# grantsrb/PyTorch-A2C

Measured on AMD Instinct MI355X. Metric: env-steps/sec (rollout+update), higher is better.
Workload: dtype f32

## Files before the change

### pytorch-a2c_amd/csrc/conv.hip

```cpp
#include <stdlib.h>
#include <algorithm>
#include <map>
#include <mutex>
#include "a2c_common.h"

bool c3_supported(const a2c_conv_desc* d, int kind);
size_t c3_prep_floats(const a2c_conv_desc* d, int kind);
int c3_prep(const a2c_conv_desc* d, int kind, const float* weight, float* out, hipStream_t st);
int c3_fwd(const a2c_conv_desc* d, const float* in, long in_bs, const float* frag, const float* bias, int relu, float* out,
           long out_bs, unsigned* signs, long signs_bs, int B, hipStream_t st);
int c3_bwd_data(const a2c_conv_desc* d, const float* dout, const float* frag, const float* mask, const unsigned* signs,
                long signs_bs, float* din, int B, hipStream_t st);
long c3_sign_words(const a2c_conv_desc* d);
bool c3_bwd_signs_supported(const a2c_conv_desc* d);
bool c3_bwd_mask_supported(const a2c_conv_desc* d);
bool c3w_supported(const a2c_conv_desc* d);
size_t c3w_ws_bytes(const a2c_conv_desc* d);
int c3w_bwd_weight(const a2c_conv_desc* d, const float* in, long in_bs, const float* dout, float* dW, float* db, int B, void* ws,
                   size_t ws_bytes, hipStream_t st);
bool c3_fwd_frames_supported(const a2c_conv_desc* d);
bool c3_chain_supported(const a2c_conv_desc* d, int n);
int c3_chain_fwd(const a2c_conv_desc* d, int n, const float* in, long in_bs, const float* const* frag, const float* const* bias,
                 int relu, float* const* out, const long* out_bs, unsigned* const* signs, const long* signs_bs, int B, hipStream_t st);
int c3_fwd_frames(const a2c_conv_desc* d, const unsigned char* f, long bs, long T, const int* nv, long nv_s, const float* frag,
// ... 2846 lines not shown
    } else {
    WS_STI(v0, 0) WS_STI(v1, 1) WS_STI(v2, 2) WS_STI(v3, 3) WS_STI(v4, 4) WS_STI(v5, 5) WS_STI(v6, 6)
    WS_STI(v7, 7) WS_STI(v8, 8) WS_STI(v9, 9) WS_STI(v10, 10) WS_STI(v11, 11) WS_STI(v12, 12) WS_STI(v13, 13)
    }
    __syncthreads();
    if (bco < p.Cout) {
      const float* __restrict__ pl = ldo + bco * p.PLANEo;
      float sb = 0.f;
      for (int i = bpart; i < NP; i += ST_NT / 16) sb += pl[i];
      dbacc += sb;
    }
#define WS_ROWS(R0, R1)                                                                                     \
    for (int rr = (R0); rr < (R1); ++rr) {                                                                  \
      const int r = 2 * rr + h;                                                                             \
      const float* __restrict__ arow = ldo + j * p.PLANEo + r * p.OW + kk;                                  \
      const float* __restrict__ brow = img + r * 4 * p.WP + boff;                                              \
      for (int c0 = 0; c0 < c4n; c0 += 5) {                                                                 \
        float av[5];                                                                                        \
        float4 bv[5];                                                                                       \
        _Pragma("unroll") for (int u = 0; u < 5; ++u) {                                                     \
          const int c4 = min(c0 + u, c4n - 1);                                                              \
          av[u] = (c0 + u < c4n) ? arow[4 * c4] : 0.f;                                                      \
          bv[u] = *reinterpret_cast<const float4*>(brow + 16 * c4);                                         \
        }                                                                                                   \
        _Pragma("unroll") for (int u = 0; u < 5; ++u) {                                                     \
          acc0 = __builtin_amdgcn_mfma_f32_16x16x4f32(av[u], bv[u].x, acc0, 0, 0, 0);                       \
          acc1 = __builtin_amdgcn_mfma_f32_16x16x4f32(av[u], bv[u].y, acc1, 0, 0, 0);                       \
          acc2 = __builtin_amdgcn_mfma_f32_16x16x4f32(av[u], bv[u].z, acc2, 0, 0, 0);                       \
          acc3 = __builtin_amdgcn_mfma_f32_16x16x4f32(av[u], bv[u].w, acc3, 0, 0, 0);                       \
        }                                                                                                   \
      }                                                                                                     \
    }
    if (U8) {
      const unsigned char* __restrict__ nus = fsrc(nn);
      nv = p.nvalid[nn];
      WS_LDD(d0, 0, ndsrc) WS_LDD(d1, 1, ndsrc) WS_LDD(d2, 2, ndsrc) WS_LDD(d3, 3, ndsrc) WS_LDU(g0, 0, nus) WS_LDU(g1, 1, nus)
      WS_ROWS(0, s1)
      WS_LDU(g2, 2, nus) WS_LDU(g3, 3, nus) WS_LDU(g4, 4, nus) WS_LDU(g5, 5, nus) WS_LDU(g6, 6, nus) WS_LDU(g7, 7, nus)
      WS_ROWS(s1, s2)
      WS_LDU(g8, 8, nus) WS_LDU(g9, 9, nus) WS_LDU(g10, 10, nus) WS_LDU(g11, 11, nus) WS_LDU(g12, 12, nus) WS_LDU(g13, 13, nus)
      WS_ROWS(s2, nrow)
    } else {
    WS_LDD(d0, 0, ndsrc) WS_LDD(d1, 1, ndsrc) WS_LDD(d2, 2, ndsrc) WS_LDD(d3, 3, ndsrc) WS_LDI(v0, 0, nsrc) WS_LDI(v1, 1, nsrc)
    WS_ROWS(0, s1)
    WS_LDI(v2, 2, nsrc) WS_LDI(v3, 3, nsrc) WS_LDI(v4, 4, nsrc) WS_LDI(v5, 5, nsrc) WS_LDI(v6, 6, nsrc) WS_LDI(v7, 7, nsrc)
    WS_ROWS(s1, s2)
    WS_LDI(v8, 8, nsrc) WS_LDI(v9, 9, nsrc) WS_LDI(v10, 10, nsrc) WS_LDI(v11, 11, nsrc) WS_LDI(v12, 12, nsrc) WS_LDI(v13, 13, nsrc)
    WS_ROWS(s2, nrow)
    }
  }
  __syncthreads();
  float* __restrict__ scr = lds;
  if (h == 1) {
    *reinterpret_cast<float4*>(scr + ((q * 4 + 0) * 64 + lane) * 4) = (float4){acc0[0], acc0[1], acc0[2], acc0[3]};
    *reinterpret_cast<float4*>(scr + ((q * 4 + 1) * 64 + lane) * 4) = (float4){acc1[0], acc1[1], acc1[2], acc1[3]};
    *reinterpret_cast<float4*>(scr + ((q * 4 + 2) * 64 + lane) * 4) = (float4){acc2[0], acc2[1], acc2[2], acc2[3]};
    *reinterpret_cast<float4*>(scr + ((q * 4 + 3) * 64 + lane) * 4) = (float4){acc3[0], acc3[1], acc3[2], acc3[3]};
  }
  float* __restrict__ red = lds + 4096;
  red[bpart * 16 + bco] = dbacc;
  __syncthreads();
  float* __restrict__ sl = p.slab + (long)blockIdx.x * ((long)p.Cout * p.K + p.Cout);
  if (h == 0) {
#pragma unroll
    for (int x = 0; x < 4; ++x) {
      const float4 o = *reinterpret_cast<const float4*>(scr + ((q * 4 + x) * 64 + lane) * 4);
      const f32x4 a = x == 0 ? acc0 : x == 1 ? acc1 : x == 2 ? acc2 : acc3;
      const float t[4] = {a[0] + o.x, a[1] + o.y, a[2] + o.z, a[3] + o.w};
#pragma unroll
      for (int rr = 0; rr < 4; ++rr) {
        const int co = 4 * kk + rr;
        if (co < p.Cout) sl[(long)co * p.K + knat + x] = t[rr];
      }
    }
  }
  if (tid < p.Cout) {
    float sb = 0.f;
    for (int x = 0; x < ST_NT / 16; ++x) sb += red[x * 16 + tid];
    sl[(long)p.Cout * p.K + tid] = sb;
  }
}

struct WsbGeo { int NG, NGT, NB, PA, PP, PLS, SK, no_ring; };
template <int DUMMY>
__global__ __launch_bounds__(ST_NT) __attribute__((amdgpu_waves_per_eu(2, 2))) void wgrad_stream_bf16_kernel(WstreamP p, WsbGeo gq) {
  extern __shared__ __attribute__((aligned(16))) float lds[];
  typedef __bf16 bf16x8w __attribute__((ext_vector_type(8)));
  unsigned short* __restrict__ A = reinterpret_cast<unsigned short*>(lds);
  unsigned short* __restrict__ P = A + 3 * 16 * gq.PA;
  const int tid = threadIdx.x, lane = tid & 63, w = tid >> 6;
  const int g = lane >> 4, j = lane & 15;
  const int HW = p.H * p.W, NP = p.OH * p.OW;
  const int w4 = p.W >> 2;
  const int dper4 = NP >> 2, dtot4 = p.Cout * dper4;
  const int NG = gq.NG, NGT = gq.NGT, NB = gq.NB, PA = gq.PA, PP = gq.PP, PLS = gq.PLS, SK = gq.SK;
  const int spr = (w4 + 1) >> 1, nslot = 4 * p.H * spr;
  {
    u32x4w* z = reinterpret_cast<u32x4w*>(lds);
    const int n16 = (3 * 16 * PA * 2 + 16 * PLS * 2) >> 4;
    for (int i = tid; i < n16; i += ST_NT) z[i] = (u32x4w){0u, 0u, 0u, 0u};
  }
  const int ky = j >> 1;
  f32x4 acc[16];
#pragma unroll
  for (int t = 0; t < 16; ++t) acc[t] = (f32x4){0.f, 0.f, 0.f, 0.f};
  float dbv[4] = {0.f, 0.f, 0.f, 0.f};
  f32x4 d0 = {}, d1 = {}, d2 = {}, d3 = {};
  uint2 g0 = {}, g1 = {}, g2 = {}, g3 = {}, g4 = {}, g5 = {}, g6 = {}, g7 = {};
  int nv = 4;
  auto fsrc = [&](long nn_) { const long r_ = nn_ / p.T; return p.fstore + r_ * p.fs_slot_stride + (nn_ - r_ * p.T) * (long)HW; };
  int soff[8];
  int sdst[8];
  unsigned int smask[8];
#pragma unroll
  for (int u = 0; u < 8; ++u) {
    const int idx = tid + u * ST_NT;
    const bool ok = idx < nslot;
    const int ii = ok ? idx : 0;
    const int c = ii / (p.H * spr), rem = ii - c * (p.H * spr), row = rem / spr, sp = rem - row * spr;
    soff[u] = (c * p.H + row) * p.W + 8 * sp;
    sdst[u] = ok ? (c * 4) * PLS + row * PP + (row >> 2) * SK + 2 * sp : -1;
    smask[u] = ((2 * sp + 1 < w4) ? 0xffffff00u : 0u) | (unsigned int)c;
  }
  int soff2[2], sdst2[2];
  unsigned int smask2[2];
#pragma unroll
  for (int u = 0; u < 2; ++u) {
    const int idx = tid + u * ST_NT;
    const bool ok = idx < p.H * spr;
    const int ii = ok ? idx : 0;
    const int row = ii / spr, sp = ii - row * spr;
    soff2[u] = (3 * p.H + row) * p.W + 8 * sp;
    sdst2[u] = ok ? row * PP + (row >> 2) * SK + 2 * sp : -1;
    smask2[u] = (2 * sp + 1 < w4) ? 1u : 0u;
  }
  int rot = 0;
  int pofs0 = 0, pofs1 = 4 * PLS, pofs2 = 8 * PLS, pofs3 = 12 * PLS;
  int adst[4];
#pragma unroll
  for (int u = 0; u < 4; ++u) {
    const int idx = tid + u * ST_NT;
    const bool ok = idx < dtot4;
    const int ii = ok ? idx : 0;
    const int co = ii / dper4, p0 = (ii - co * dper4) << 2;
    const int r = p0 / p.OW, c = p0 - r * p.OW;
    adst[u] = ok ? co * PA + (r * NG + (c >> 3)) * 8 + (c & 7) : -1;
  }
  const bool ring_off = gq.no_ring != 0;
  const long chunk = (p.B + gridDim.x - 1) / gridDim.x;
  long n = (long)blockIdx.x * chunk;
  const long n_end = n + chunk < (long)p.B ? n + chunk : (long)p.B;
#define WSB_LDU(var, u, src)                                                                                   \
  {                                                                                                            \
    const unsigned int* s_ = reinterpret_cast<const unsigned int*>((src) + soff[u]);                            \
    var.x = s_[0];                                                                                             \
    var.y = s_[(smask[u] >> 8) ? 1 : 0];                                                                       \
  }
#define WSB_LOADD(NN, D0, D1, D2, D3)                                                                          \
  {                                                                                                            \
    const float* __restrict__ ds_ = p.dout + (NN) * (long)p.Cout * NP;                                         \
    D0 = *reinterpret_cast<const f32x4*>(ds_ + (min(tid + 0 * ST_NT, dtot4 - 1) << 2));                        \
    D1 = *reinterpret_cast<const f32x4*>(ds_ + (min(tid + 1 * ST_NT, dtot4 - 1) << 2));                        \
    D2 = *reinterpret_cast<const f32x4*>(ds_ + (min(tid + 2 * ST_NT, dtot4 - 1) << 2));                        \
    D3 = *reinterpret_cast<const f32x4*>(ds_ + (min(tid + 3 * ST_NT, dtot4 - 1) << 2));                        \
  }
#define WSB_LDU2(var, u, src)                                                                                  \
  {                                                                                                            \
    const unsigned int* s_ = reinterpret_cast<const unsigned int*>((src) + soff2[u]);                           \
    var.x = s_[0];                                                                                             \
    var.y = s_[smask2[u] ? 1 : 0];                                                                             \
  }
#define WSB_LOADG(NN, INC_)                                                                                    \
  {                                                                                                            \
    const unsigned char* __restrict__ us_ = fsrc(NN);                                                          \
    if (INC_) {                                                                                                \
      WSB_LDU2(g0, 0, us_) WSB_LDU2(g1, 1, us_)                                                                \
    } else {                                                                                                   \
      WSB_LDU(g0, 0, us_) WSB_LDU(g1, 1, us_) WSB_LDU(g2, 2, us_) WSB_LDU(g3, 3, us_)                          \
      WSB_LDU(g4, 4, us_) WSB_LDU(g5, 5, us_) WSB_LDU(g6, 6, us_) WSB_LDU(g7, 7, us_)                          \
    }                                                                                                          \
  }
#define WSB_STD(var, u)                                                                                        \
  if (adst[u] >= 0) {                                                                                          \
    const float e_[4] = {var.x, var.y, var.z, var.w};                                                          \
    unsigned short pc_[3][4];                                                                                  \
    _Pragma("unroll") for (int i_ = 0; i_ < 4; ++i_) {                                                        \
      const __bf16 h0_ = (__bf16)e_[i_];                                                                       \
      const float r1_ = e_[i_] - (float)h0_;                                                                   \
      const __bf16 h1_ = (__bf16)r1_;                                                                          \
      const float r2_ = r1_ - (float)h1_;                                                                      \
      pc_[0][i_] = __builtin_bit_cast(unsigned short, h0_);                                                    \
      pc_[1][i_] = __builtin_bit_cast(unsigned short, h1_);                                                    \
      pc_[2][i_] = __builtin_bit_cast(unsigned short, (__bf16)r2_);                                            \
    }                                                                                                          \
    dbv[u] += (e_[0] + e_[1]) + (e_[2] + e_[3]);                                                               \
    unsigned short* a_ = A + adst[u];                                                                          \
    _Pragma("unroll") for (int pc = 0; pc < 3; ++pc)                                                          \
      *reinterpret_cast<uint2*>(a_ + pc * 16 * PA) = make_uint2((unsigned int)pc_[pc][0] | ((unsigned int)pc_[pc][1] << 16), \
                                                                (unsigned int)pc_[pc][2] | ((unsigned int)pc_[pc][3] << 16)); \
  }
#define WSB_STU(var, u)                                                                                        \
  if (sdst[u] >= 0) {                                                                                          \
    const int c_ = (int)(smask[u] & 0xffu);                                                                    \
    const unsigned int x0_ = c_ < 4 - nv ? 0u : var.x, x1_ = (c_ < 4 - nv || !(smask[u] >> 8)) ? 0u : var.y;   \
    unsigned int* d_ = reinterpret_cast<unsigned int*>(P + sdst[u]);                                           \
    const int ps_ = PLS >> 1;                                                                                  \
    d_[0] = __builtin_amdgcn_perm(__float_as_uint((float)(x1_ & 0xffu)), __float_as_uint((float)(x0_ & 0xffu)), 0x07060302u); \
    d_[ps_] = __builtin_amdgcn_perm(__float_as_uint((float)((x1_ >> 8) & 0xffu)), __float_as_uint((float)((x0_ >> 8) & 0xffu)), 0x07060302u); \
    d_[2 * ps_] = __builtin_amdgcn_perm(__float_as_uint((float)((x1_ >> 16) & 0xffu)), __float_as_uint((float)((x0_ >> 16) & 0xffu)), 0x07060302u); \
    d_[3 * ps_] = __builtin_amdgcn_perm(__float_as_uint((float)(x1_ >> 24)), __float_as_uint((float)(x0_ >> 24)), 0x07060302u); \
  }
  auto matrix = [&]() {
    for (int b = w; b < NB; b += ST_NT / 64) {
      const int grp = 4 * b + g;
      const unsigned short* __restrict__ ap = A + j * PA + grp * 8;
      const bf16x8w ah = *reinterpret_cast<const bf16x8w*>(ap);
      const bf16x8w am = *reinterpret_cast<const bf16x8w*>(ap + 16 * PA);
      const bf16x8w al = *reinterpret_cast<const bf16x8w*>(ap + 32 * PA);
      const int gcl = min(grp, NGT - 1);
      const int r = gcl / NG, gc = gcl - r * NG;
      const unsigned short* __restrict__ bp = P + (j & 1) * PLS + (4 * r + ky) * PP + (r + (ky >> 2)) * SK + 8 * gc;
#pragma unroll
      for (int t = 0; t < 16; ++t) {
        const int ci = t >> 2, kxh = (t >> 1) & 1, kp = t & 1;
        const int po = ci == 0 ? pofs0 : ci == 1 ? pofs1 : ci == 2 ? pofs2 : pofs3;
        const unsigned short* __restrict__ bx = bp + po + 2 * kp * PLS;
        const uint2 lo = *reinterpret_cast<const uint2*>(bx), hi = *reinterpret_cast<const uint2*>(bx + 4);
        u32x4w o;
        if (kxh) {
          const unsigned int nx = *reinterpret_cast<const unsigned int*>(bx + 8);
          o[0] = __builtin_amdgcn_alignbit(lo.y, lo.x, 16u);
          o[1] = __builtin_amdgcn_alignbit(hi.x, lo.y, 16u);
          o[2] = __builtin_amdgcn_alignbit(hi.y, hi.x, 16u);
          o[3] = __builtin_amdgcn_alignbit(nx, hi.y, 16u);
        } else {
          o[0] = lo.x; o[1] = lo.y; o[2] = hi.x; o[3] = hi.y;
        }
        const bf16x8w bv = __builtin_bit_cast(bf16x8w, o);
        acc[t] = __builtin_amdgcn_mfma_f32_16x16x32_bf16(ah, bv, acc[t], 0, 0, 0);
        acc[t] = __builtin_amdgcn_mfma_f32_16x16x32_bf16(am, bv, acc[t], 0, 0, 0);
        acc[t] = __builtin_amdgcn_mfma_f32_16x16x32_bf16(al, bv, acc[t], 0, 0, 0);
      }
    }
  };
#define WSB_STU2(var, u, PB_)                                                                                  \
  if (sdst2[u] >= 0) {                                                                                         \
    const unsigned int x0_ = var.x, x1_ = smask2[u] ? var.y : 0u;                                              \
    unsigned int* d_ = reinterpret_cast<unsigned int*>(P + (PB_) + sdst2[u]);                                  \
    const int ps_ = PLS >> 1;                                                                                  \
    d_[0] = __builtin_amdgcn_perm(__float_as_uint((float)(x1_ & 0xffu)), __float_as_uint((float)(x0_ & 0xffu)), 0x07060302u); \
    d_[ps_] = __builtin_amdgcn_perm(__float_as_uint((float)((x1_ >> 8) & 0xffu)), __float_as_uint((float)((x0_ >> 8) & 0xffu)), 0x07060302u); \
    d_[2 * ps_] = __builtin_amdgcn_perm(__float_as_uint((float)((x1_ >> 16) & 0xffu)), __float_as_uint((float)((x0_ >> 16) & 0xffu)), 0x07060302u); \
    d_[3 * ps_] = __builtin_amdgcn_perm(__float_as_uint((float)(x1_ >> 24)), __float_as_uint((float)(x0_ >> 24)), 0x07060302u); \
  }
  auto succ = [&](long a_, long b_, int nva_, int nvb_) {
    return !ring_off && b_ == a_ + 1 && (b_ % p.T) != 0 && nvb_ == 4 && nva_ >= 3;
  };
#define WSB_ITER(N_, D0, D1, D2, D3)                                                                           \
  {                                                                                                            \
    const long n2_ = ((N_) + 2 < n_end) ? (N_) + 2 : (N_);                                                     \
    const long n1_ = ((N_) + 1 < n_end) ? (N_) + 1 : (N_);                                                     \
    __syncthreads();                                  \
    if (inc_cur) rot = (rot + 1) & 3; else rot = 0;                                                            \
    pofs0 = rot * 4 * PLS; pofs1 = ((rot + 1) & 3) * 4 * PLS; pofs2 = ((rot + 2) & 3) * 4 * PLS; pofs3 = ((rot + 3) & 3) * 4 * PLS; \
    WSB_STD(D0, 0) WSB_STD(D1, 1) WSB_STD(D2, 2) WSB_STD(D3, 3)                                                \
    if (inc_cur) {                                                                                             \
      WSB_STU2(g0, 0, pofs3) WSB_STU2(g1, 1, pofs3)                                                            \
    } else {                                                                                                   \
      WSB_STU(g0, 0) WSB_STU(g1, 1) WSB_STU(g2, 2) WSB_STU(g3, 3) WSB_STU(g4, 4) WSB_STU(g5, 5) WSB_STU(g6, 6) WSB_STU(g7, 7) \
    }                                                                                                          \
    __syncthreads();                                                                                           \
                     \
    inc_cur = n1_ != (N_) && succ((N_), n1_, nv, nv1);                                                         \
    nv = nv1;                                             \
    WSB_LOADG(n1_, inc_cur)                                                                                    \
    nv1 = p.nvalid[n2_];                                                                                       \
    WSB_LOADD(n2_, D0, D1, D2, D3)                                                                             \
    matrix();                                                                                                  \
  }
  f32x4 e0 = {}, e1 = {}, e2 = {}, e3 = {};
  bool inc_cur = false;
  int nv1 = 4;
  if (n < n_end) {
    const long n1 = (n + 1 < n_end) ? n + 1 : n;
    WSB_LOADD(n, d0, d1, d2, d3)
    nv = p.nvalid[n];
    WSB_LOADG(n, false)
    nv1 = p.nvalid[n1];
    WSB_LOADD(n1, e0, e1, e2, e3)
  }
  for (; n < n_end; n += 2) {
    WSB_ITER(n, d0, d1, d2, d3)
    if (n + 1 < n_end) WSB_ITER(n + 1, e0, e1, e2, e3)
  }
#undef WSB_ITER
#undef WSB_STU2
#undef WSB_LDU2
#undef WSB_LOADD
#undef WSB_LOADG
#undef WSB_LDU
#undef WSB_STD
#undef WSB_STU
  float* __restrict__ sl = p.slab + (long)blockIdx.x * ((long)p.Cout * p.K + p.Cout);
  float* __restrict__ scr = lds;
#pragma unroll
  for (int t0 = 0; t0 < 16; t0 += 4) {
    __syncthreads();
#pragma unroll
    for (int x = 0; x < 4; ++x)
      *reinterpret_cast<float4*>(scr + ((w * 4 + x) * 64 + lane) * 4) = (float4){acc[t0 + x][0], acc[t0 + x][1], acc[t0 + x][2], acc[t0 + x][3]};
    __syncthreads();
#pragma unroll
    for (int e = 0; e < 2; ++e) {
      const int o = tid + e * ST_NT, x = o >> 8, l = (o >> 2) & 63, rr = o & 3;
      float v = scr[((0 * 4 + x) * 64 + l) * 4 + rr];
#pragma unroll
      for (int ww = 1; ww < ST_NT / 64; ++ww) v += scr[((ww * 4 + x) * 64 + l) * 4 + rr];
      const int t = t0 + x, ci = t >> 2, kxh = (t >> 1) & 1, kp = t & 1;
      const int jj = l & 15, co = 4 * (l >> 4) + rr;
      const int k = ((ci * 8 + (jj >> 1)) * 8) + 4 * kxh + 2 * kp + (jj & 1);
      if (co < p.Cout) sl[(long)co * p.K + k] = v;
    }
  }
  __syncthreads();
  float* __restrict__ red = lds;
#pragma unroll
  for (int u = 0; u < 4; ++u) red[tid + u * ST_NT] = dbv[u];
  __syncthreads();
  if (tid < p.Cout) {
    float sb = 0.f;
    for (int i = tid * dper4; i < (tid + 1) * dper4; ++i) sb += red[i];
    sl[(long)p.Cout * p.K + tid] = sb;
  }
}

static bool plan_wstream_bf16(const a2c_conv_desc* d, const WstreamP& p, WsbGeo& gq, size_t& lds) {
  gq.NG = (d->OW + 7) / 8;
  gq.no_ring = a2c_env_on("A2C_WSB_NO_RING");
  gq.NGT = d->OH * gq.NG;
  gq.NB = (gq.NGT + 3) / 4;
  const int need_dw = gq.NB * 16;
  int pa_dw = ((need_dw + 31) / 32) * 32 + 4;
  if (pa_dw - 32 >= need_dw) pa_dw -= 32;
  gq.PA = pa_dw * 2;
  gq.PP = gq.NG * 8 + 8;
  gq.SK = 4;
  gq.PLS = d->H * gq.PP + (d->H / 4 + 1) * gq.SK + 24;
  if (d->W / 4 > gq.NG * 8 + 1 || d->OW % 4 || d->Cout > 16) return false;
  lds = (size_t)3 * 16 * gq.PA * 2 + (size_t)16 * gq.PLS * 2;
  lds = (lds + 15) / 16 * 16;
  if (lds < 4 * (size_t)(8 * 4 * 256) || 4 * d->H * ((d->W / 4 + 1) / 2) > 8 * ST_NT) return false;
  if ((long)d->Cout * (d->OH * d->OW / 4) > 4L * ST_NT) return false;
  (void)p;
  return lds <= 160 * 1024 && (gq.PP * 2) % 8 == 0 && (gq.PLS * 2) % 8 == 0 && 4 * (d->OH - 1) + 7 < d->H;
}

static bool plan_wstream(const a2c_conv_desc* d, WstreamP& p) {
  if (!(d->ks == 8 && d->stride == 4 && d->pad == 0 && d->Cin == 4 && d->Cout <= 16 && d->W % 4 == 0 && d->OW % 4 == 0)) return false;
  const int NP = d->OH * d->OW;
  p.H = d->H; p.W = d->W; p.OH = d->OH; p.OW = d->OW; p.Cout = d->Cout; p.K = d->Cin * 64;
  p.WP = d->W;
  p.PLANE1 = ((d->H * p.WP + 63) / 64) * 64;
  p.PLANEo = ((NP + 31) / 32) * 32 + 2;
  if (d->H * d->W > ST_NS * ST_NT || d->Cout * NP > 4 * ST_NT * 4 || d->OH < 6) return false;
  if (4 * p.PLANE1 < 4096 + 512) return false;
  return 4 * (size_t)(4 * p.PLANE1 + 16 * p.PLANEo) <= 160 * 1024;
}
static int stream_grid() {
  static const int n_cu = []() { int dev = 0, n = 0; (void)hipGetDevice(&dev);
                                 (void)hipDeviceGetAttribute(&n, hipDeviceAttributeMultiprocessorCount, dev); return n > 0 ? n : 256; }();
  return n_cu;
}

__global__ __launch_bounds__(256) void wgrad_reduce_kernel(const float* __restrict__ slab, int nslab, long per,
                                                           long nW, float* __restrict__ dW, float* __restrict__ db) {
  for (long i = blockIdx.x * 256L + threadIdx.x; i < per; i += gridDim.x * 256L) {
    float s = 0.f;
    int z = 0;
    for (; z + 8 <= nslab; z += 8) {
      float t[8];
#pragma unroll
      for (int u = 0; u < 8; ++u) t[u] = slab[(long)(z + u) * per + i];
#pragma unroll
      for (int u = 0; u < 8; ++u) s += t[u];
    }
    for (; z < nslab; ++z) s += slab[(long)z * per + i];
    if (i < nW) dW[i] = s;
    else if (db) db[i - nW] = s;
  }
}

struct WgradPlan { SrcTile t; int OWp, PLANEo, MT, KTW, grid, run, rs, pf, ex; size_t lds; };

#define WGRAD_PF_A 1, 3, true, 4, 16, true
#define WGRAD_PF_C 2, 4, false, 12, 8, true
#define WGRAD_PF_D 2, 4, false, 14, 8, true, 2, 1
#define WGRAD_VARIANTS(X)                                                                                      \
  if (pl.pf == 2) { X(WGRAD_PF_D); }                                                                           \
  else if (pl.pf && pl.KTW == 3) { X(WGRAD_PF_A); }                                                            \
  else if (pl.pf) { X(WGRAD_PF_C); }                                                                           \
  else if (pl.rs && pl.KTW == 3) { X(1, 3, true, 0, 0, true); }                                                \
  else if (pl.rs) { X(2, 9, true, 0, 0, true); }                                                               \
  else if (pl.MT == 1 && pl.KTW == 1) { X(1, 1, false, 0, 0, true); }                                         \
  else if (pl.MT == 1 && pl.KTW == 4) { X(1, 4); }                                                            \
  else if (pl.MT == 2 && pl.KTW == 4 && pl.ex) { X(2, 4, false, 0, 0, true); }                                \
  else if (pl.MT == 2 && pl.KTW == 4) { X(2, 4); }                                                            \
  else if (pl.KTW == 5) { X(4, 5, false, 0, 0, true); }                                                       \
  else if (pl.ex) { X(4, 7, false, 0, 0, true); }                                                              \
  else { X(4, 7); }

static const void* wgrad_fn(const WgradPlan& pl) {
#define WGRAD_FN(...) return (const void*)wgrad_kernel<__VA_ARGS__>
  WGRAD_VARIANTS(WGRAD_FN)
#undef WGRAD_FN
}

static int wgrad_run_variant(const a2c_conv_desc* d) {
  if (!run_layout(d)) return 0;
  const int mt = ceil_div(d->Cout, 16), c4n = ceil_div(d->OW, 4), rgs = d->Cin * d->ks * 2 / 16;
  if (d->stride == 4 && mt == 1 && rgs == 4 && c4n == 5) return 1;
  if (d->stride == 2 && mt == 2 && rgs == 8 && c4n == 3) return 2;
  return 0;
}
// ... 818 lines not shown
    if (rc != A2C_OK) return rc;
  }
  return A2C_OK;
}
}
extern "C" {

size_t a2c_conv2d_bwd_data_w1_ws_bytes(const a2c_conv_desc* d2, const a2c_conv_desc* d1, int B) {
  BandW1Plan pl;
  if (B < 1 || !plan_band_w1(d2, d1, B, nullptr, pl)) return 0;
  int grid = 0;
  for (int v : {1, 2, 4}) {
    if (d2->OW % v) continue;
    pl.vec = v;
    const int g = band_w1_grid(pl, B);
    if (g > grid) grid = g;
  }
  return (size_t)grid * ((size_t)d1->Cout * d1->Cin * 9 + d1->Cout) * sizeof(float);
}

int a2c_conv2d_bwd_data_w1(const a2c_conv_desc* d2, const float* dout, const float* wprep_bwd, const float* mask,
                           const a2c_conv_desc* d1, const float* x, int64_t x_bstride, float* dW1, float* db1, int B,
                           void* ws, size_t ws_bytes, a2c_stream_t stream) {
  if (B < 1 || !dout || !wprep_bwd || !mask || !x || !dW1 || !db1) return A2C_ERR_ARG;
  BandW1Plan pl;
  if (((uintptr_t)mask % 16) || ((uintptr_t)x % 16) || x_bstride % 4 || !plan_band_w1(d2, d1, B, dout, pl)) return A2C_ERR_ARG;
  pl.q2.b.wfrag = wprep_bwd; pl.q2.b.mask = mask; pl.q2.b.din = nullptr;
  pl.fw.x = x; pl.fw.x_bs = x_bstride; pl.fw.slab = (float*)ws;
  const int grid = band_w1_grid(pl, B);
  const size_t per = (size_t)d1->Cout * pl.fw.K1 + d1->Cout;
  if (grid < 1) return A2C_ERR_ARG;
  if (!ws || ws_bytes < (size_t)grid * per * sizeof(float)) return A2C_ERR_WORKSPACE;
  hipStream_t st = a2c_s(stream);
#define W1_LAUNCH(V_, P_)                                                                                         \
  if (pl.vec == V_ && pl.pfb == P_)                                                                               \
    hipLaunchKernelGGL((bwd_band2_kernel<1, V_, P_, true>), dim3(grid), dim3(256), pl.lds, st, pl.q2, pl.fw);
  BAND_W1_CASES(W1_LAUNCH)
#undef W1_LAUNCH
  A2C_CHECK_LAUNCH();
  const long nW = (long)d1->Cout * pl.fw.K1;
  hipLaunchKernelGGL(wgrad_reduce_kernel, dim3(a2c_grid_1d((long)per, 256)), dim3(256), 0, st, (const float*)ws, grid,
                     (long)per, nW, dW1, db1);
  A2C_CHECK_LAUNCH();
  return A2C_OK;
}

size_t a2c_conv2d_bwd_weight_ws_bytes(const a2c_conv_desc* d, int B) {
  WgradPlan pl, pg;
  if (!desc_ok(d) || B < 0 || !plan_wgrad(d, B, pl) || !plan_wgrad(d, B, pg, false)) return 0;
  int grid = pl.grid > pg.grid ? pl.grid : pg.grid;
  WstreamP wp;
  if (plan_wstream(d, wp) && stream_grid() > grid) grid = stream_grid();
  const size_t base = (size_t)grid * ((size_t)d->Cout * d->Cin * d->ks * d->ks + d->Cout) * sizeof(float);
  const size_t c3 = c3w_ws_bytes(d);
  return c3 > base ? c3 : base;
}

int a2c_conv2d_bwd_weight_frames(const a2c_conv_desc* d, const uint8_t* fstore, int64_t slot_stride, int64_t T,
                                 const int* nvalid, const float* dout, float* dW, float* db, int B, void* ws, size_t ws_bytes,
                                 a2c_stream_t stream) {
  if (!desc_ok(d) || B < 1 || !fstore || !nvalid || !dout || !dW || T < 1) return A2C_ERR_ARG;
  if (c3w_supported(d) && d->Cin == 4) {
    if (((uintptr_t)fstore % 4) || slot_stride % 4 || ((uintptr_t)dout % 16) || ((uintptr_t)dW % 16) || ((uintptr_t)ws % 16) ||
        slot_stride < (T + 3) * (int64_t)d->H * d->W)
      return A2C_ERR_ARG;
    if (!ws || ws_bytes < a2c_conv2d_bwd_weight_ws_bytes(d, B)) return A2C_ERR_WORKSPACE;
    return c3w_bwd_weight_frames(d, fstore, (long)slot_stride, (long)T, nvalid, dout, dW, db, B, ws, ws_bytes, a2c_s(stream));
  }
  WstreamP wp;
  if (!plan_wstream(d, wp) || (d->H * d->W) % 16 || ((uintptr_t)fstore % 16) || slot_stride % 16 || ((uintptr_t)dout % 16) ||
      slot_stride < (T + 3) * (int64_t)d->H * d->W)
    return A2C_ERR_ARG;
  if (!ws || ws_bytes < a2c_conv2d_bwd_weight_ws_bytes(d, B)) return A2C_ERR_WORKSPACE;
  hipStream_t st = a2c_s(stream);
  const int grid = stream_grid();
  wp.in = nullptr; wp.in_bs = 0; wp.dout = dout; wp.slab = (float*)ws; wp.B = B;
  wp.fstore = fstore; wp.fs_slot_stride = (long)slot_stride; wp.T = (int)T; wp.nvalid = nvalid;
  {
    WsbGeo gq;
    size_t ldsb = 0;
    if (!a2c_env_on("A2C_WGRAD_F32") && plan_wstream_bf16(d, wp, gq, ldsb)) {
      static bool attrb = false;
      if (!attrb) {
        if (hipFuncSetAttribute((const void*)wgrad_stream_bf16_kernel<0>, hipFuncAttributeMaxDynamicSharedMemorySize, 160 * 1024) != hipSuccess)
          return A2C_ERR_LAUNCH;
        attrb = true;
      }
      const int gb = grid < B ? grid : B;
      hipLaunchKernelGGL(wgrad_stream_bf16_kernel<0>, dim3(gb), dim3(ST_NT), ldsb, st, wp, gq);
      A2C_CHECK_LAUNCH();
      const long nWb = (long)wp.Cout * wp.K, perb = nWb + wp.Cout;
      hipLaunchKernelGGL(wgrad_reduce_kernel, dim3(a2c_grid_1d(perb, 256)), dim3(256), 0, st, (const float*)ws, gb, perb, nWb, dW, db);
      A2C_CHECK_LAUNCH();
      return A2C_OK;
    }
  }
  const size_t lds = 4 * (size_t)(4 * wp.PLANE1 + 16 * wp.PLANEo);
  static bool attr = false;
  if (!attr) {
    if (hipFuncSetAttribute((const void*)wgrad_stream_kernel<true>, hipFuncAttributeMaxDynamicSharedMemorySize, 160 * 1024) != hipSuccess)
      return A2C_ERR_LAUNCH;
    attr = true;
  }
  hipLaunchKernelGGL(wgrad_stream_kernel<true>, dim3(grid < B ? grid : B), dim3(ST_NT), lds, st, wp);
  A2C_CHECK_LAUNCH();
  const int g = grid < B ? grid : B;
  const long nWs = (long)wp.Cout * wp.K, pers = nWs + wp.Cout;
  hipLaunchKernelGGL(wgrad_reduce_kernel, dim3(a2c_grid_1d(pers, 256)), dim3(256), 0, st, (const float*)ws, g, pers, nWs, dW, db);
  A2C_CHECK_LAUNCH();
  return A2C_OK;
}

int a2c_conv2d_bwd_weight_rank(const a2c_conv_desc* d, const float* in, int64_t in_bstride, const float* dl, int64_t ld_dl,
                               int n_logits, const float* Wc, const uint8_t* maskbits, int64_t mask_row_bytes, float* dW, float* db,
                               int B, void* ws, size_t ws_bytes, a2c_stream_t stream) {
  if (!desc_ok(d) || B < 1 || !in || !dl || !Wc || !maskbits || !dW || !db) return A2C_ERR_ARG;
  if (in_bstride % 4 || ((uintptr_t)in % 16) || ld_dl < n_logits || mask_row_bytes < (int64_t)d->Cout * d->OH * d->OW / 8 ||
      in_bstride < (int64_t)d->Cin * d->H * d->W || !a2c_conv2d_bwd_rank_supported(d, n_logits, B))
    return A2C_ERR_ARG;
  if (!ws || ws_bytes < a2c_conv2d_bwd_weight_ws_bytes(d, B)) return A2C_ERR_WORKSPACE;
  WgradPlan pl;
  if (!plan_wgrad(d, B, pl, true)) return A2C_ERR_ARG;
  const int grid = stream_grid() < pl.grid ? stream_grid() : pl.grid;
  hipStream_t st = a2c_s(stream);
  static bool attrr = false;
  if (!attrr) {
    if (hipFuncSetAttribute((const void*)wgrad_x6_kernel<true>, hipFuncAttributeMaxDynamicSharedMemorySize, wx::LDS_BYTES) != hipSuccess)
      return A2C_ERR_LAUNCH;
    attrr = true;
  }
  WgradX6P xp;
  xp.in = in; xp.in_bs = (long)in_bstride; xp.dout = nullptr; xp.slab = (float*)ws; xp.B = B;
  xp.dl = dl; xp.ldl = (long)ld_dl; xp.nlog = n_logits; xp.Wc = Wc; xp.a2b = maskbits; xp.a2b_row = (long)mask_row_bytes;
  hipLaunchKernelGGL(wgrad_x6_kernel<true>, dim3(grid), dim3(wx::NT), wx::LDS_BYTES, st, xp);
  A2C_CHECK_LAUNCH();
  const long nWx = 32L * 256, perx = nWx + 32;
  hipLaunchKernelGGL(wgrad_reduce_kernel, dim3(a2c_grid_1d(perx, 256)), dim3(256), 0, st, (const float*)ws, grid, perx, nWx, dW, db);
  A2C_CHECK_LAUNCH();
  return A2C_OK;
}

int a2c_conv2d_bwd_weight(const a2c_conv_desc* d, const float* in, int64_t in_bstride, const float* dout, float* dW,
                          float* db, int B, void* ws, size_t ws_bytes, a2c_stream_t stream) {
  WgradPlan pl;
  if (!desc_ok(d) || B < 1 || !in || !dout || !dW) return A2C_ERR_ARG;
  const bool aligned = (in_bstride % 4 == 0) && ((uintptr_t)in % 16 == 0) && ((uintptr_t)dout % 8 == 0);
  if (!plan_wgrad(d, B, pl, aligned)) return A2C_ERR_ARG;
  if (!ws || ws_bytes < a2c_conv2d_bwd_weight_ws_bytes(d, B)) return A2C_ERR_WORKSPACE;
  hipStream_t st = a2c_s(stream);
  if (c3w_supported(d) && aligned && ((uintptr_t)dout % 16 == 0) && ((uintptr_t)dW % 16 == 0) && ((uintptr_t)ws % 16 == 0))
    return c3w_bwd_weight(d, in, (long)in_bstride, dout, dW, db, B, ws, ws_bytes, st);
  {
    WstreamP wp;
    const int grid = stream_grid();
    if (aligned && B >= 8 * grid && ((uintptr_t)dout % 16 == 0) && !a2c_env_on("A2C_NO_STREAM") &&
        plan_wstream(d, wp)) {
      wp.in = in; wp.in_bs = in_bstride; wp.dout = dout; wp.slab = (float*)ws; wp.B = B;
      wp.fstore = nullptr; wp.fs_slot_stride = 0; wp.T = 1; wp.nvalid = nullptr;
      const size_t lds = 4 * (size_t)(4 * wp.PLANE1 + 16 * wp.PLANEo);
      static bool attr = false;
      if (!attr) {
        if (hipFuncSetAttribute((const void*)wgrad_stream_kernel<false>, hipFuncAttributeMaxDynamicSharedMemorySize, 160 * 1024) != hipSuccess)
          return A2C_ERR_LAUNCH;
        attr = true;
      }
      hipLaunchKernelGGL(wgrad_stream_kernel<false>, dim3(grid), dim3(ST_NT), lds, st, wp);
      A2C_CHECK_LAUNCH();
      const long nWs = (long)wp.Cout * wp.K, pers = nWs + wp.Cout;
      hipLaunchKernelGGL(wgrad_reduce_kernel, dim3(a2c_grid_1d(pers, 256)), dim3(256), 0, st, (const float*)ws, grid, pers, nWs,
                         dW, db);
      A2C_CHECK_LAUNCH();
      return A2C_OK;
// ... 59 lines not shown
```

Before: 10.07 million.

## Software-pipeline LDS reads in bf16 weight-grad MFMA loop with inline asm waits

Replaces the generic matrix() loop in the bf16 streaming weight-gradient kernel with a compile-time-unrolled pipeline. It prefetches A and B fragments from LDS with explicit ds_read instructions and uses fine-grained lgkmcnt waits so LDS latency overlaps the MFMA work. It also recomputes whole-frame staging addresses on the fly instead of keeping eight per-thread slot arrays and eight preloaded registers, which cuts register pressure. The old path stays selectable through an env var. The risks are fragile hand-scheduled waits, a new cap on block count that can reject some shapes, and extra code size from specialising each block count.

```diff
diff --git a/pytorch-a2c_amd/csrc/conv.hip b/pytorch-a2c_amd/csrc/conv.hip
--- a/pytorch-a2c_amd/csrc/conv.hip
+++ b/pytorch-a2c_amd/csrc/conv.hip
@@ -2952,7 +2952,31 @@
 }
 
 struct WsbGeo { int NG, NGT, NB, PA, PP, PLS, SK, no_ring; };
-template <int DUMMY>
+constexpr int WSB_MAXBLK = 4;
+typedef void __attribute__((address_space(3)))* wsb_lptr_t;
+__device__ __forceinline__ unsigned int wsb_lds_addr(const void* q) { return (unsigned int)(unsigned long)(wsb_lptr_t)q; }
+template <int OFF>
+__device__ __forceinline__ void wsb_read_a(u32x4w& v, unsigned int a) {
+  asm volatile("ds_read_b128 %0, %1 offset:%2" : "=v"(v) : "v"(a), "n"(OFF) : "memory");
+}
+__device__ __forceinline__ void wsb_read_b(u32x4w& v, unsigned int& t, unsigned int a) {
+  asm volatile("ds_read2_b64 %0, %1 offset1:1" : "=v"(v) : "v"(a) : "memory");
+  asm volatile("ds_read_b32 %0, %1 offset:16" : "=v"(t) : "v"(a) : "memory");
+}
+template <int N>
+__device__ __forceinline__ void wsb_wait(u32x4w& v, unsigned int& t) {
+  asm volatile("s_waitcnt lgkmcnt(%2)" : "+v"(v), "+v"(t) : "n"(N) : "memory");
+  __builtin_amdgcn_sched_barrier(0);
+}
+template <int N>
+__device__ __forceinline__ void wsb_wait(u32x4w& v, unsigned int& t, u32x4w& a0, u32x4w& a1, u32x4w& a2) {
+  asm volatile("s_waitcnt lgkmcnt(%5)" : "+v"(v), "+v"(t), "+v"(a0), "+v"(a1), "+v"(a2) : "n"(N) : "memory");
+  __builtin_amdgcn_sched_barrier(0);
+}
+template <int V>
+struct WsbC { static constexpr int value = V; };
+
+template <int SERIAL>
 __global__ __launch_bounds__(ST_NT) __attribute__((amdgpu_waves_per_eu(2, 2))) void wgrad_stream_bf16_kernel(WstreamP p, WsbGeo gq) {
   extern __shared__ __attribute__((aligned(16))) float lds[];
   typedef __bf16 bf16x8w __attribute__((ext_vector_type(8)));
@@ -2976,22 +3000,9 @@
   for (int t = 0; t < 16; ++t) acc[t] = (f32x4){0.f, 0.f, 0.f, 0.f};
   float dbv[4] = {0.f, 0.f, 0.f, 0.f};
   f32x4 d0 = {}, d1 = {}, d2 = {}, d3 = {};
-  uint2 g0 = {}, g1 = {}, g2 = {}, g3 = {}, g4 = {}, g5 = {}, g6 = {}, g7 = {};
+  uint2 g0 = {}, g1 = {};
   int nv = 4;
   auto fsrc = [&](long nn_) { const long r_ = nn_ / p.T; return p.fstore + r_ * p.fs_slot_stride + (nn_ - r_ * p.T) * (long)HW; };
-  int soff[8];
-  int sdst[8];
-  unsigned int smask[8];
-#pragma unroll
-  for (int u = 0; u < 8; ++u) {
-    const int idx = tid + u * ST_NT;
-    const bool ok = idx < nslot;
-    const int ii = ok ? idx : 0;
-    const int c = ii / (p.H * spr), rem = ii - c * (p.H * spr), row = rem / spr, sp = rem - row * spr;
-    soff[u] = (c * p.H + row) * p.W + 8 * sp;
-    sdst[u] = ok ? (c * 4) * PLS + row * PP + (row >> 2) * SK + 2 * sp : -1;
-    smask[u] = ((2 * sp + 1 < w4) ? 0xffffff00u : 0u) | (unsigned int)c;
-  }
   int soff2[2], sdst2[2];
   unsigned int smask2[2];
 #pragma unroll
@@ -3020,12 +3031,6 @@
   const long chunk = (p.B + gridDim.x - 1) / gridDim.x;
   long n = (long)blockIdx.x * chunk;
   const long n_end = n + chunk < (long)p.B ? n + chunk : (long)p.B;
-#define WSB_LDU(var, u, src)                                                                                   \
-  {                                                                                                            \
-    const unsigned int* s_ = reinterpret_cast<const unsigned int*>((src) + soff[u]);                            \
-    var.x = s_[0];                                                                                             \
-    var.y = s_[(smask[u] >> 8) ? 1 : 0];                                                                       \
-  }
 #define WSB_LOADD(NN, D0, D1, D2, D3)                                                                          \
   {                                                                                                            \
     const float* __restrict__ ds_ = p.dout + (NN) * (long)p.Cout * NP;                                         \
@@ -3041,14 +3046,9 @@
     var.y = s_[smask2[u] ? 1 : 0];                                                                             \
   }
 #define WSB_LOADG(NN, INC_)                                                                                    \
-  {                                                                                                            \
+  if (INC_) {                                                                                                  \
     const unsigned char* __restrict__ us_ = fsrc(NN);                                                          \
-    if (INC_) {                                                                                                \
-      WSB_LDU2(g0, 0, us_) WSB_LDU2(g1, 1, us_)                                                                \
-    } else {                                                                                                   \
-      WSB_LDU(g0, 0, us_) WSB_LDU(g1, 1, us_) WSB_LDU(g2, 2, us_) WSB_LDU(g3, 3, us_)                          \
-      WSB_LDU(g4, 4, us_) WSB_LDU(g5, 5, us_) WSB_LDU(g6, 6, us_) WSB_LDU(g7, 7, us_)                          \
-    }                                                                                                          \
+    WSB_LDU2(g0, 0, us_) WSB_LDU2(g1, 1, us_)                                                                  \
   }
 #define WSB_STD(var, u)                                                                                        \
   if (adst[u] >= 0) {                                                                                          \
@@ -3069,17 +3069,97 @@
       *reinterpret_cast<uint2*>(a_ + pc * 16 * PA) = make_uint2((unsigned int)pc_[pc][0] | ((unsigned int)pc_[pc][1] << 16), \
                                                                 (unsigned int)pc_[pc][2] | ((unsigned int)pc_[pc][3] << 16)); \
   }
-#define WSB_STU(var, u)                                                                                        \
-  if (sdst[u] >= 0) {                                                                                          \
-    const int c_ = (int)(smask[u] & 0xffu);                                                                    \
-    const unsigned int x0_ = c_ < 4 - nv ? 0u : var.x, x1_ = (c_ < 4 - nv || !(smask[u] >> 8)) ? 0u : var.y;   \
-    unsigned int* d_ = reinterpret_cast<unsigned int*>(P + sdst[u]);                                           \
-    const int ps_ = PLS >> 1;                                                                                  \
-    d_[0] = __builtin_amdgcn_perm(__float_as_uint((float)(x1_ & 0xffu)), __float_as_uint((float)(x0_ & 0xffu)), 0x07060302u); \
-    d_[ps_] = __builtin_amdgcn_perm(__float_as_uint((float)((x1_ >> 8) & 0xffu)), __float_as_uint((float)((x0_ >> 8) & 0xffu)), 0x07060302u); \
-    d_[2 * ps_] = __builtin_amdgcn_perm(__float_as_uint((float)((x1_ >> 16) & 0xffu)), __float_as_uint((float)((x0_ >> 16) & 0xffu)), 0x07060302u); \
-    d_[3 * ps_] = __builtin_amdgcn_perm(__float_as_uint((float)(x1_ >> 24)), __float_as_uint((float)(x0_ >> 24)), 0x07060302u); \
-  }
+  auto whole = [&](long nn_, int nv_) __attribute__((always_inline)) {
+    const unsigned char* __restrict__ us_ = fsrc(nn_);
+    const int hs_ = p.H * spr;
+    int tid_ = tid;
+    asm volatile("" : "+v"(tid_));
+    uint2 f_[8];
+#pragma unroll
+    for (int u = 0; u < 8; ++u) {
+      const int idx = tid_ + u * ST_NT;
+      const int ii = idx < nslot ? idx : 0;
+      const int c = ii / hs_, rem = ii - c * hs_, row = rem / spr, sp = rem - row * spr;
+      const unsigned int* s_ = reinterpret_cast<const unsigned int*>(us_ + (c * p.H + row) * p.W + 8 * sp);
+      f_[u].x = s_[0];
+      f_[u].y = s_[(2 * sp + 1 < w4) ? 1 : 0];
+    }
+#pragma unroll
+    for (int u = 0; u < 8; ++u) {
+      const int idx = tid_ + u * ST_NT;
+      if (idx < nslot) {
+        const int c = idx / hs_, rem = idx - c * hs_, row = rem / spr, sp = rem - row * spr;
+        const unsigned int x0_ = c < 4 - nv_ ? 0u : f_[u].x, x1_ = (c < 4 - nv_ || 2 * sp + 1 >= w4) ? 0u : f_[u].y;
+        unsigned int* d_ = reinterpret_cast<unsigned int*>(P + (c * 4) * PLS + row * PP + (row >> 2) * SK + 2 * sp);
+        const int ps_ = PLS >> 1;
+        d_[0] = __builtin_amdgcn_perm(__float_as_uint((float)(x1_ & 0xffu)), __float_as_uint((float)(x0_ & 0xffu)), 0x07060302u);
+        d_[ps_] = __builtin_amdgcn_perm(__float_as_uint((float)((x1_ >> 8) & 0xffu)), __float_as_uint((float)((x0_ >> 8) & 0xffu)), 0x07060302u);
+        d_[2 * ps_] = __builtin_amdgcn_perm(__float_as_uint((float)((x1_ >> 16) & 0xffu)), __float_as_uint((float)((x0_ >> 16) & 0xffu)), 0x07060302u);
+        d_[3 * ps_] = __builtin_amdgcn_perm(__float_as_uint((float)(x1_ >> 24)), __float_as_uint((float)(x0_ >> 24)), 0x07060302u);
+      }
+    }
+  };
+  const int wu = __builtin_amdgcn_readfirstlane(w);
+  const int nbw = NB > wu ? (NB - wu + ST_NT / 64 - 1) / (ST_NT / 64) : 0;
+  const unsigned int aad = wsb_lds_addr(A + j * PA + (4 * w + g) * 8);
+  unsigned int bad[WSB_MAXBLK];
+#pragma unroll
+  for (int k = 0; k < WSB_MAXBLK; ++k) {
+    const int gcl = min(4 * (w + k * (ST_NT / 64)) + g, NGT - 1);
+    const int r = gcl / NG, gc = gcl - r * NG;
+    bad[k] = wsb_lds_addr(P + (j & 1) * PLS + (4 * r + ky) * PP + (r + (ky >> 2)) * SK + 8 * gc);
+  }
+  auto pipe = [&](auto NBW_) __attribute__((always_inline)) {
+    constexpr int nbk = decltype(NBW_)::value;
+    if constexpr (nbk == 0) return;
+    const int sb[8] = {2 * pofs0, 2 * (pofs0 + 2 * PLS), 2 * pofs1, 2 * (pofs1 + 2 * PLS),
+                       2 * pofs2, 2 * (pofs2 + 2 * PLS), 2 * pofs3, 2 * (pofs3 + 2 * PLS)};
+    const unsigned int a1o = 32u * (unsigned int)PA, a2o = 64u * (unsigned int)PA;
+    u32x4w af[2][3];
+    u32x4w bq[3];
+    unsigned int bt[3];
+    wsb_read_a<0>(af[0][0], aad);
+    wsb_read_a<0>(af[0][1], aad + a1o);
+    wsb_read_a<0>(af[0][2], aad + a2o);
+    wsb_read_b(bq[0], bt[0], bad[0] + sb[0]);
+    wsb_read_b(bq[1], bt[1], bad[0] + sb[1]);
+    auto stage = [&](auto K_, auto S_, auto LAST_) __attribute__((always_inline)) {
+      constexpr int k = decltype(K_)::value, s = decltype(S_)::value, gs = 8 * k + s;
+      constexpr bool last = decltype(LAST_)::value != 0;
+      constexpr int kn = k + 1 < WSB_MAXBLK ? k + 1 : k;
+      if constexpr (s + 2 < 8) wsb_read_b(bq[(gs + 2) % 3], bt[(gs + 2) % 3], bad[k] + sb[s + 2]);
+      else if constexpr (!last) wsb_read_b(bq[(gs + 2) % 3], bt[(gs + 2) % 3], bad[kn] + sb[s + 2 - 8]);
+      if constexpr (s == 5 && !last) {
+        wsb_read_a<512 * kn>(af[kn & 1][0], aad);
+        wsb_read_a<512 * kn>(af[kn & 1][1], aad + a1o);
+        wsb_read_a<512 * kn>(af[kn & 1][2], aad + a2o);
+      }
+      constexpr int nw = s < 5 ? 4 : last ? 2 * (7 - s) : 7;
+      if constexpr (s == 0) wsb_wait<nw>(bq[gs % 3], bt[gs % 3], af[k & 1][0], af[k & 1][1], af[k & 1][2]);
+      else wsb_wait<nw>(bq[gs % 3], bt[gs % 3]);
+      const u32x4w v = bq[gs % 3];
+      const u32x4w o = {__builtin_amdgcn_alignbit(v[1], v[0], 16u), __builtin_amdgcn_alignbit(v[2], v[1], 16u),
+                        __builtin_amdgcn_alignbit(v[3], v[2], 16u), __builtin_amdgcn_alignbit(bt[gs % 3], v[3], 16u)};
+      const bf16x8w b0 = __builtin_bit_cast(bf16x8w, v), b1 = __builtin_bit_cast(bf16x8w, o);
+      constexpr int t0 = (s >> 1) * 4 + (s & 1), t1 = t0 + 2;
+#pragma unroll
+      for (int pc = 0; pc < 3; ++pc) {
+        const bf16x8w a = __builtin_bit_cast(bf16x8w, af[k & 1][pc]);
+        acc[t0] = __builtin_amdgcn_mfma_f32_16x16x32_bf16(a, b0, acc[t0], 0, 0, 0);
+        acc[t1] = __builtin_amdgcn_mfma_f32_16x16x32_bf16(a, b1, acc[t1], 0, 0, 0);
+      }
+    };
+#define WSB_BLOCK(K_, L_)                                                                                      \
+    stage(WsbC<K_>{}, WsbC<0>{}, WsbC<L_>{}); stage(WsbC<K_>{}, WsbC<1>{}, WsbC<L_>{});                        \
+    stage(WsbC<K_>{}, WsbC<2>{}, WsbC<L_>{}); stage(WsbC<K_>{}, WsbC<3>{}, WsbC<L_>{});                        \
+    stage(WsbC<K_>{}, WsbC<4>{}, WsbC<L_>{}); stage(WsbC<K_>{}, WsbC<5>{}, WsbC<L_>{});                        \
+    stage(WsbC<K_>{}, WsbC<6>{}, WsbC<L_>{}); stage(WsbC<K_>{}, WsbC<7>{}, WsbC<L_>{});
+    WSB_BLOCK(0, (nbk == 1))
+    if constexpr (nbk > 1) { WSB_BLOCK(1, (nbk == 2)) }
+    if constexpr (nbk > 2) { WSB_BLOCK(2, (nbk == 3)) }
+    if constexpr (nbk > 3) { WSB_BLOCK(3, 1) }
+#undef WSB_BLOCK
+  };
   auto matrix = [&]() {
     for (int b = w; b < NB; b += ST_NT / 64) {
       const int grp = 4 * b + g;
@@ -3137,40 +3217,47 @@
     if (inc_cur) {                                                                                             \
       WSB_STU2(g0, 0, pofs3) WSB_STU2(g1, 1, pofs3)                                                            \
     } else {                                                                                                   \
-      WSB_STU(g0, 0) WSB_STU(g1, 1) WSB_STU(g2, 2) WSB_STU(g3, 3) WSB_STU(g4, 4) WSB_STU(g5, 5) WSB_STU(g6, 6) WSB_STU(g7, 7) \
+      whole((N_), nv);                                                                                         \
     }                                                                                                          \
     __syncthreads();                                                                                           \
                      \
-    inc_cur = n1_ != (N_) && succ((N_), n1_, nv, nv1);                                                         \
-    nv = nv1;                                             \
+    const int nv1_ = __builtin_amdgcn_readfirstlane(nv1);  \
+    inc_cur = n1_ != (N_) && succ((N_), n1_, nv, nv1_);                                                        \
+    nv = nv1_;                                                                                                 \
     WSB_LOADG(n1_, inc_cur)                                                                                    \
-    nv1 = p.nvalid[n2_];                                                                                       \
+    nv1 = p.nvalid[n2_ + lz];                                                                                  \
     WSB_LOADD(n2_, D0, D1, D2, D3)                                                                             \
-    matrix();                                                                                                  \
+    if constexpr (SERIAL != 0) matrix(); else pipe(NBW_);                                                      \
   }
   f32x4 e0 = {}, e1 = {}, e2 = {}, e3 = {};
   bool inc_cur = false;
+  int lz = 0;
+  asm volatile("" : "+v"(lz));
   int nv1 = 4;
   if (n < n_end) {
     const long n1 = (n + 1 < n_end) ? n + 1 : n;
     WSB_LOADD(n, d0, d1, d2, d3)
     nv = p.nvalid[n];
-    WSB_LOADG(n, false)
-    nv1 = p.nvalid[n1];
+    nv1 = p.nvalid[n1 + lz];
     WSB_LOADD(n1, e0, e1, e2, e3)
   }
-  for (; n < n_end; n += 2) {
-    WSB_ITER(n, d0, d1, d2, d3)
-    if (n + 1 < n_end) WSB_ITER(n + 1, e0, e1, e2, e3)
-  }
+  auto run = [&](auto NBW_) __attribute__((always_inline)) {
+    for (; n < n_end; n += 2) {
+      WSB_ITER(n, d0, d1, d2, d3)
+      if (n + 1 < n_end) WSB_ITER(n + 1, e0, e1, e2, e3)
+    }
+  };
+  if (SERIAL != 0 || nbw == 2) run(WsbC<2>{});
+  else if (nbw == 1) run(WsbC<1>{});
+  else if (nbw == 0) run(WsbC<0>{});
+  else if (nbw == 3) run(WsbC<3>{});
+  else run(WsbC<4>{});
 #undef WSB_ITER
 #undef WSB_STU2
 #undef WSB_LDU2
 #undef WSB_LOADD
 #undef WSB_LOADG
-#undef WSB_LDU
 #undef WSB_STD
-#undef WSB_STU
   float* __restrict__ sl = p.slab + (long)blockIdx.x * ((long)p.Cout * p.K + p.Cout);
   float* __restrict__ scr = lds;
 #pragma unroll
@@ -3209,6 +3296,7 @@
   gq.no_ring = a2c_env_on("A2C_WSB_NO_RING");
   gq.NGT = d->OH * gq.NG;
   gq.NB = (gq.NGT + 3) / 4;
+  if (gq.NB > WSB_MAXBLK * (ST_NT / 64)) return false;
   const int need_dw = gq.NB * 16;
   int pa_dw = ((need_dw + 31) / 32) * 32 + 4;
   if (pa_dw - 32 >= need_dw) pa_dw -= 32;
@@ -4193,12 +4281,16 @@
     if (!a2c_env_on("A2C_WGRAD_F32") && plan_wstream_bf16(d, wp, gq, ldsb)) {
       static bool attrb = false;
       if (!attrb) {
-        if (hipFuncSetAttribute((const void*)wgrad_stream_bf16_kernel<0>, hipFuncAttributeMaxDynamicSharedMemorySize, 160 * 1024) != hipSuccess)
+        if (hipFuncSetAttribute((const void*)wgrad_stream_bf16_kernel<0>, hipFuncAttributeMaxDynamicSharedMemorySize, 160 * 1024) != hipSuccess ||
+            hipFuncSetAttribute((const void*)wgrad_stream_bf16_kernel<1>, hipFuncAttributeMaxDynamicSharedMemorySize, 160 * 1024) != hipSuccess)
           return A2C_ERR_LAUNCH;
         attrb = true;
       }
       const int gb = grid < B ? grid : B;
-      hipLaunchKernelGGL(wgrad_stream_bf16_kernel<0>, dim3(gb), dim3(ST_NT), ldsb, st, wp, gq);
+      if (a2c_env_on("A2C_WSB_SERIAL"))
+        hipLaunchKernelGGL(wgrad_stream_bf16_kernel<1>, dim3(gb), dim3(ST_NT), ldsb, st, wp, gq);
+      else
+        hipLaunchKernelGGL(wgrad_stream_bf16_kernel<0>, dim3(gb), dim3(ST_NT), ldsb, st, wp, gq);
       A2C_CHECK_LAUNCH();
       const long nWb = (long)wp.Cout * wp.K, perb = nWb + wp.Cout;
       hipLaunchKernelGGL(wgrad_reduce_kernel, dim3(a2c_grid_1d(perb, 256)), dim3(256), 0, st, (const float*)ws, gb, perb, nWb, dW, db);
```

After: 10.23 million, median of 4. +1.6%, better.
